# zengyf131/gswt_renderer

Measured on AMD Instinct MI355X. Metric: frames/sec @1920x1080, 32x32 Wang-tile grid, higher is better.
Workload: dtype f32

## Files before the change

gswt_renderer_amd/_lib.py:

```python
from __future__ import annotations

import ctypes as C
import os

_HERE = os.path.dirname(os.path.abspath(__file__))
LIB_PATH = os.environ.get("GSWT_HIP_LIB") or os.path.join(_HERE, "lib", "libgswt_hip.so")

GSWT_OK = 0
GSWT_ERR_BAD_ARG = -1
GSWT_ERR_CAPACITY = -2
GSWT_ERR_HIP = -3
GSWT_ERR_STATE = -4
GSWT_ERR_RCCL = -6
GSWT_COMM_ID_BYTES = 128
GSWT_ORDER_REFERENCE = 0
GSWT_ORDER_DEPTH = 1
GSWT_OPT_NO_LOD_PREFILTER = 1
GSWT_OPT_DEBUG_VARYINGS = 2
GSWT_OPT_SEGMENT = 3
GSWT_DEFAULT_SEGMENT = 1536
GSWT_OPT_DEBUG_FLAGS = 4
GSWT_OPT_TIMING = 5
GSWT_OPT_PAIR_CAP = 6
GSWT_OPT_NO_MERGE_REUSE = 7
GSWT_OPT_DEFER_SWAP = 8
GSWT_OPT_GRAPH = 9
GSWT_OPT_STRICT_VS = 10
GSWT_OPT_DEPTH_PASSES = 12
GSWT_OPT_COMPOSITE = 13
GSWT_OPT_DEPTH_SORT = 14
GSWT_OPT_NO_CHUNK_CULL = 15
GSWT_OPT_ITEM_ORDER = 16
GSWT_OPT_PROJECTION = 17
GSWT_PROJECTION_PERSPECTIVE, GSWT_PROJECTION_ORTHO = 0, 1
GSWT_OPT_ANTIALIAS = 18
GSWT_SCENE_TEX = 0
GSWT_SCENE_RAW_DEPTH = 1
GSWT_SCENE_RAW_TABLES = 2
GSWT_SCENE_STATIC_LIST = 3
GSWT_SCENE_STATIC_BOXES = 4
GSWT_SCENE_LISTS = 5
GSWT_SCENE_BOUNDS = 6
GSWT_SHARD_ROWS = 0
GSWT_SHARD_COLUMNS = 1
GSWT_OUT_RGBA32F = 0
GSWT_OUT_RGBA8_UNORM = 1
GSWT_OUT_BGRA8_UNORM = 2
GSWT_VIDEO_NV12 = 16
GSWT_VIDEO_I420 = 17
GSWT_PROXY_SRC_RGBA8 = 0
GSWT_PROXY_SRC_RGBA16 = 1


class CameraUniforms(C.Structure):
    _fields_ = [("projection", C.c_float * 16), ("view", C.c_float * 16), ("focal", C.c_float * 2),
                ("viewport", C.c_float * 2), ("htan_fov", C.c_float * 4), ("cam_pos", C.c_float * 4)]


class SceneUniforms(C.Structure):
    _fields_ = [("splat_scale", C.c_float), ("tile_width", C.c_float), ("use_clip", C.c_uint32),
                ("clip_height", C.c_float), ("surface_type", C.c_uint32), ("sphere_radius", C.c_float),
                ("point_cloud_radius", C.c_float), ("transition_width_ratio", C.c_float),
                ("num_lod", C.c_uint32), ("draw_mode", C.c_uint32), ("map_half_wh", C.c_uint32 * 2),
                ("center_coord", C.c_int32 * 2), ("_pad0", C.c_uint32 * 2),
                ("transition_dist_vec", C.c_float * 16), ("height_map_scale", C.c_float * 4),
                ("scene_scale", C.c_float * 4)]


# ... 187 lines not shown
```

gswt_renderer_amd/csrc/gswt_api.hip:

```cpp
#include "gswt_ctx.h"
#include "host/gswt_surface.h"

#include <algorithm>
#include <limits>
#include <memory>

using namespace gswt;


static int finish_frame(gswt_ctx* c, FrameSlot& sl);

void gswt::collect_slot(gswt_ctx* c, FrameSlot& sl)
{
    if (!sl.pending || sl.collected) return;
    sl.collected_rc = finish_frame(c, sl);
    sl.collected_timings = c->timings;
    sl.collected = true;
}

hipError_t gswt::collect_pending(gswt_ctx* c)
{
    for (auto& sl : c->slots) collect_slot(c, sl);
    return sync_all(c);
}
// ... 94 lines not shown
    if (c->own_stream && c->stream) hipStreamDestroy(c->stream);
    if (hip_stream) { c->stream = (hipStream_t)hip_stream; c->own_stream = false; return GSWT_OK; }
    c->stream = nullptr; c->own_stream = true;
    hipSetDevice(c->device);
    HIP_TRY(c, hipStreamCreateWithFlags(&c->stream, hipStreamNonBlocking));
    return GSWT_OK;
} GSWT_CATCH

int gswt_set_option(gswt_ctx* c, int key, int value)
try {
    if (!c) return GSWT_ERR_BAD_ARG;
    switch (key) {
    case GSWT_OPT_NO_LOD_PREFILTER: c->opt.no_prefilter = value; c->draws_ready = false; return GSWT_OK;
    case GSWT_OPT_DEBUG_VARYINGS: c->opt.debug_varyings = value; return GSWT_OK;
    case GSWT_OPT_DEBUG_FLAGS:
        if (value != 0) return fail(c, GSWT_ERR_BAD_ARG, "GSWT_OPT_DEBUG_FLAGS is reserved: only 0 is accepted");
        return GSWT_OK;
    case GSWT_OPT_TIMING: c->opt.timing = value; return GSWT_OK;
    case GSWT_OPT_NO_MERGE_REUSE: c->opt.no_merge_reuse = value; return GSWT_OK;
    case GSWT_OPT_DEFER_SWAP: c->opt.defer_swap = value; return GSWT_OK;
    case GSWT_OPT_GRAPH: c->opt.graph = value; return GSWT_OK;
    case GSWT_OPT_STRICT_VS: c->opt.strict_vs = value != 0; return GSWT_OK;
    case GSWT_OPT_PROJECTION:
        if (value != 0 && value != 1) return fail(c, GSWT_ERR_BAD_ARG, "GSWT_OPT_PROJECTION: 0 (perspective) or 1 (orthographic), not %d", value);
        c->opt.projection = value; return GSWT_OK;
    case GSWT_OPT_ANTIALIAS:
        if (value < 0 || value > 4096) return fail(c, GSWT_ERR_BAD_ARG, "GSWT_OPT_ANTIALIAS: 0 (off) or 1..4096 (filter variance in 1/1024 px^2), not %d", value);
        c->opt.antialias = value; return GSWT_OK;
    case GSWT_OPT_COMPOSITE:
        if (value < 0 || value > 2) return fail(c, GSWT_ERR_BAD_ARG, "unknown compositor variant %d", value);
        c->opt.composite = value; return GSWT_OK;
    case GSWT_OPT_NO_CHUNK_CULL: c->opt.no_chunk_cull = value != 0; return GSWT_OK;
    case GSWT_OPT_ITEM_ORDER: c->opt.item_order = value != 0; return GSWT_OK;
    case GSWT_OPT_DEPTH_SORT:
        if (value < 0 || value > 2) return fail(c, GSWT_ERR_BAD_ARG, "GSWT_OPT_DEPTH_SORT: 0 (auto), 1 (global passes) or 2 (tile-local)");
        c->opt.depth_sort = value; c->depth_max_tile_len = 0;
        return GSWT_OK;
    case GSWT_OPT_DEPTH_PASSES:
        if (value < 1 || value > 4) return fail(c, GSWT_ERR_BAD_ARG, "depth-sort passes must be 1..4");
        c->depth_passes = (uint32_t)value; c->depth_passes_low_run = 0;
        return GSWT_OK;
    case GSWT_OPT_PAIR_CAP:
        if (value < 0) return fail(c, GSWT_ERR_BAD_ARG, "pair capacity must be >= 0");
        c->opt.fixed_pair_cap = value > 0; if (value > 0) c->pair_cap = (uint32_t)value;
        return GSWT_OK;
    case GSWT_OPT_SEGMENT:
        if (value < 256 || value % 256) return fail(c, GSWT_ERR_BAD_ARG, "segment must be a positive multiple of 256");
        c->opt.segment = value; return GSWT_OK;
    default: return fail(c, GSWT_ERR_BAD_ARG, "unknown option %d", key);
    }
} GSWT_CATCH

int gswt_set_atmosphere(gswt_ctx* c, const gswt_atmosphere* a)
try {
    if (!c) return GSWT_ERR_BAD_ARG;
    if (!a) { c->atm = gswt_atmosphere{}; return GSWT_OK; }
    const float inf = std::numeric_limits<float>::infinity();
    const struct { const char* name; float v; } fields[] = {
        {"fade_start", a->fade_start}, {"fade_end", a->fade_end}, {"fog_density", a->fog_density}, {"fog_start", a->fog_start},
        {"fog_max", a->fog_max}, {"fog_color[0]", a->fog_color[0]}, {"fog_color[1]", a->fog_color[1]}, {"fog_color[2]", a->fog_color[2]}};
    for (const auto& fd : fields)
        if (!(std::fabs(fd.v) < inf)) return fail(c, GSWT_ERR_BAD_ARG, "gswt_set_atmosphere: %s = %g is not finite", fd.name, fd.v);
    if (a->fade_start != 0.0f || a->fade_end != 0.0f) {
        if (!(a->fade_start >= 0.0f)) return fail(c, GSWT_ERR_BAD_ARG, "gswt_set_atmosphere: fade_start = %g, not >= 0", a->fade_start);
        if (!(a->fade_end > a->fade_start))
            return fail(c, GSWT_ERR_BAD_ARG, "gswt_set_atmosphere: fade_end = %g, not above fade_start = %g", a->fade_end, a->fade_start);
// ... 218 lines not shown
    if (!sl.live_cnt.p) { HIP_TRY(c, sl.live_cnt.ensure(16 * kSuperStride)); HIP_TRY(c, hipMemsetAsync(sl.live_cnt.p, 0, sl.live_cnt.cap * 4, sl.stream)); }
    HIP_TRY(c, sl.draw_culled.ensure_roomy((size_t)D.n_draws + 1));
    HIP_TRY(c, sl.cell_culled.ensure((size_t)b.n_cells + 1));
    if (a.su.draw_mode != 0u) HIP_TRY(c, sl.col_f.ensure(n_slots_all + 1));
    if (need_depths) HIP_TRY(c, sl.depths.ensure(n_slots_all + 1));
    if (c->opt.debug_varyings) HIP_TRY(c, c->dbg.ensure((size_t)D.n_entries + 1));
    const size_t range_words = 2 * (nt + 1), list_words = tile_depth_list_words(nt);
    auto uint2s = [](size_t words) { return (words + 1) / 2 + 1; };
    HIP_TRY(c, sl.ranges.ensure(range_words / 2 + 2 * uint2s(list_words)));
    b.n_zero_ranges = (uint32_t)(range_words + list_words + 1);
    const size_t counter_words = 16, n_super = (size_t)D.n_chunks / 256 + 1;
    const size_t super_words = (2 * (size_t)kSuperStride + 1) * n_super;
    const size_t rw_pair = radix_ws_words(cap, key_bits), rw_depth = depth_bits ? radix_ws_words(cap, depth_bits) : 0;
    HIP_TRY(c, sl.ghist.ensure_roomy(counter_words + super_words + rw_pair + rw_depth + 16));
    b.n_zero_head = (uint32_t)(counter_words + super_words + radix_ws_zero_words(cap, key_bits));
    b.n_zero_depth = depth_bits ? (uint32_t)radix_ws_zero_words(cap, depth_bits) : 0u;
    HIP_TRY(c, sl.keys_a.ensure_roomy((size_t)cap + 1)); HIP_TRY(c, sl.keys_b.ensure_roomy((size_t)cap + 1));
    HIP_TRY(c, sl.vals_a.ensure_roomy((size_t)cap + 1)); HIP_TRY(c, sl.vals_b.ensure_roomy((size_t)cap + 1));
    if (depth_order) { HIP_TRY(c, sl.aux_a.ensure_roomy((size_t)cap + 1)); HIP_TRY(c, sl.aux_b.ensure_roomy((size_t)cap + 1)); }
    HIP_TRY(c, sl.item_base.ensure_roomy(nt + 2));
    HIP_TRY(c, sl.partials.ensure_roomy((nt + cap / seg + 1) * 256));
    if (a.d_out_depth) HIP_TRY(c, sl.partials_z.ensure_roomy((nt + cap / seg + 1) * 256));
    if (a.d_out_pick) HIP_TRY(c, sl.partials_pick.ensure_roomy((nt + cap / seg + 1) * 256));
    HIP_TRY(c, sl.item_tab.ensure_roomy(nt + cap / seg + 2));

    b.draws = D.draws; b.n_chunks = D.n_chunks; b.chunk_tab = D.chunk_tab.p; b.chunk_tab_xcd = D.chunk_tab_xcd.p;
    b.static_list = c->static_list.p; b.merged_list = D.merged_list.p; b.merged_map = D.merged_map.p;
    b.tex = c->tex.p; b.hmap = c->hmap.p; b.boxes = c->static_boxes.p;
    b.bg_rgba = a.d_bg; b.bg_depth = a.d_bgd; b.out = a.d_out; b.out_depth = a.d_out_depth; b.host_counters = sl.hc_dev;
    b.out_pick = reinterpret_cast<uint4*>(a.d_out_pick);
    b.n_tiles = (uint32_t)n_tiles; b.pair_cap = cap; b.seg = seg;
    b.rects = sl.rects.p; b.recs = sl.recs.p; b.depths = need_depths ? sl.depths.p : nullptr; b.col_f = sl.col_f.p; b.dbg = c->dbg.p;
    b.draw_culled = sl.draw_culled.p; b.cell_culled = sl.cell_culled.p;
    b.live_cnt = sl.live_cnt.p; b.live_cid = sl.live_cid.p; b.live_tab = sl.live_tab.p; b.block_sums = sl.block_sums.p;
    b.counters = reinterpret_cast<unsigned long long*>(sl.ghist.p);
    b.krange = reinterpret_cast<uint32_t*>(b.counters + 5);
    b.super_sums = sl.ghist.p + counter_words;
    b.radix_pair = b.super_sums + super_words;
    b.radix_depth = b.radix_pair + rw_pair;
    b.keys_a = sl.keys_a.p; b.keys_b = sl.keys_b.p; b.vals_a = sl.vals_a.p; b.vals_b = sl.vals_b.p; b.aux_a = sl.aux_a.p; b.aux_b = sl.aux_b.p;
    b.ranges = sl.ranges.p;
    b.long_tiles = reinterpret_cast<uint32_t*>(sl.ranges.p) + range_words;
    b.item_base = sl.item_base.p; b.item_tab = sl.item_tab.p; b.partials = sl.partials.p; b.partials_z = a.d_out_depth ? sl.partials_z.p : nullptr;
    b.partials_pick = a.d_out_pick ? sl.partials_pick.p : nullptr;
    const bool time_pick = a.d_out_pick != nullptr && c->opt.timing >= 1;
    b.ev_pick_begin = time_pick ? sl.ev[kEvPickBegin] : nullptr; b.ev_pick_end = time_pick ? sl.ev[kEvPickEnd] : nullptr;
    sl.pick_timed = time_pick && n_tiles > 0;
    return GSWT_OK;
}

static int emit_and_sort(gswt_ctx* c, const FrameSlot& sl, const Frame& f, const FrameBufs& b, int key_bits, const uint32_t** sorted)
{
    hipStream_t s = sl.stream;
    const uint32_t n_launch = c->opt.debug_varyings ? 0u : sl.n_launch_eff;
    const unsigned long long* const n_pairs = b.counters + 1;
    const uint32_t cap = b.pair_cap;
    if (sl.args.cfg.order_mode != GSWT_ORDER_DEPTH) {
        launch_emit(s, f, b, b.keys_a, nullptr, nullptr, n_launch);
        if (c->opt.timing >= 2) HIP_TRY(c, hipEventRecord(sl.ev[kEvEmitted], s));
        const int where = launch_sort(s, b.keys_a, b.vals_a, b.keys_b, b.vals_b, cap, n_pairs, key_bits, b.radix_pair, b.ranges);
        *sorted = where ? b.vals_b : b.vals_a;
    } else if (sl.depth_local) {
        launch_emit(s, f, b, b.keys_a, b.aux_a, nullptr, n_launch);
        if (c->opt.timing >= 2) HIP_TRY(c, hipEventRecord(sl.ev[kEvEmitted], s));
        const int where = launch_sort(s, b.keys_a, b.vals_a, b.keys_b, b.vals_b, cap, n_pairs, key_bits, b.radix_pair, b.ranges, nullptr, b.aux_a, b.aux_b);
        uint32_t* const vals = where ? b.vals_b : b.vals_a;
        launch_tile_depth_sort(s, b.ranges, vals, where ? b.aux_b : b.aux_a, where ? b.vals_a : b.vals_b, where ? b.aux_a : b.aux_b, (int)b.n_tiles,
// ... 35 lines not shown
    sl.depth_passes = depth_order ? std::min<uint32_t>(std::max<uint32_t>(c->depth_passes, 1u), 4u) : 0u;
    sl.depth_local = depth_order && c->opt.depth_sort != 1;
    if (depth_order) (sl.depth_local ? c->stat_depth_local : c->stat_depth_global)++;
    FrameBufs b;
    int rc = plan_frame_buffers(c, sl, D, f, n_tiles, sl.cap, key_bits, sl.depth_local ? 0 : 8 * (int)sl.depth_passes, b);
    if (rc != GSWT_OK) return rc;
    if (hipStreamQuery(c->stream) != hipSuccess) {
        HIP_TRY(c, hipEventRecord(sl.ev_in, c->stream));
        HIP_TRY(c, hipStreamWaitEvent(s, sl.ev_in, 0));
    }
    if (D.ev_up && D.ev_up_pending && !D.built) {
        if (hipEventQuery(D.ev_up) == hipSuccess) D.built = true;
        else HIP_TRY(c, hipStreamWaitEvent(s, D.ev_up, 0));
    }
    if (g.world > 1 && out_px > 0) HIP_TRY(c, hipMemsetAsync(a.d_out, 0, g.bytes, s));
    if (g.world > 1 && out_px > 0 && a.d_out_depth) HIP_TRY(c, hipMemsetAsync(a.d_out_depth, 0, out_px * sizeof(float), s));
    if (g.world > 1 && out_px > 0 && a.d_out_pick) HIP_TRY(c, hipMemsetAsync(a.d_out_pick, 0, out_px * sizeof(gswt_pick), s));
    const bool use_graph = c->opt.graph != 0 && c->opt.timing == 0 && !dbg && n_tiles > 0 && sl.hc_dev != nullptr;
    struct RecorderScope {
        explicit RecorderScope(GraphRec* r) { if (r) { r->n = 0; r->overflow = false; } graph_recorder() = r; }
        ~RecorderScope() { graph_recorder() = nullptr; }
    } recorder_scope(use_graph ? &sl.grec : nullptr);
    hipEvent_t* ev = sl.ev;
    if (c->opt.timing >= 1) HIP_TRY(c, hipEventRecord(ev[kEvStart], s));
    launch_cull(s, f, b, c->opt.no_chunk_cull == 0 && !dbg);
    {
        uint64_t eff = D.n_launch;
        if (!dbg && !sl.full_grid && c->live_hint) {
            const uint64_t cut = 8ull * ((uint64_t)c->live_hint + c->live_hint / 2 + 256);
            if (cut * 2 <= eff) eff = cut;
        }
        sl.n_launch_eff = (uint32_t)eff;
    }
    launch_project(s, f, b, sl.n_launch_eff, dbg, a.strict_vs, a.ortho);
    if (c->opt.timing >= 2) HIP_TRY(c, hipEventRecord(ev[kEvProjected], s));
    const uint32_t* vals = nullptr;
    rc = emit_and_sort(c, sl, f, b, key_bits, &vals);
    if (rc != GSWT_OK) return rc;
    if (c->opt.timing >= 2) HIP_TRY(c, hipEventRecord(ev[kEvSorted], s));
    if (c->opt.timing >= 2) HIP_TRY(c, hipEventRecord(ev[kEvRanges], s));
    launch_composite(s, f, b, vals, out_rows, c->opt.composite, depth_order && !sl.depth_local ? b.krange : nullptr, sl.depth_passes, depth_order,
                     c->opt.item_order != 0, c->opt.timing >= 1 ? ev[kEvCompositeBegin] : nullptr, c->opt.timing >= 1 ? ev[kEvCompositeEnd] : nullptr,
                     (int)a.cfg.out_format);
    c->last_n_tiles = (uint32_t)n_tiles;
    c->last_slot = (int)(&sl - c->slots);
    if (c->opt.timing >= 1) HIP_TRY(c, hipEventRecord(ev[kEvEnd], s));
    if (use_graph) {
        graph_recorder() = nullptr;
        const int grc = replay_graph(c, sl);
        if (grc != GSWT_OK) return grc;
    }
    HIP_TRY(c, hipGetLastError());
    if (n_tiles == 0 || !sl.hc_dev) HIP_TRY(c, hipMemcpyAsync(sl.hc, b.counters, 5 * sizeof(unsigned long long), hipMemcpyDeviceToHost, s));
    HIP_TRY(c, hipEventRecord(ev[kEvDone], s));
    sl.timing_level = c->opt.timing;
    return GSWT_OK;
}

static int finish_frame(gswt_ctx* c, FrameSlot& sl)
{
    for (int attempt = 0;; attempt++) {
        HIP_TRY(c, hipEventSynchronize(sl.ev[kEvDone]));
        const unsigned long long P64 = sl.hc[1];
        if (P64 >= 0xFFFFFF00ull) return fail(c, GSWT_ERR_CAPACITY, "gswt_render: %llu pairs exceed 2^32", P64);
        if (sl.hc[3] == 0 && P64 <= sl.cap) break;
        if (attempt >= 3) return fail(c, GSWT_ERR_CAPACITY, "gswt_render: pair capacity did not converge");
// ... 349 lines not shown
```

gswt_renderer_amd/csrc/gswt_ctx.h:

```cpp
#pragma once

#include "../../include/gswt_hip.h"
#include "gswt_device.h"

#include <cstdarg>
#include <cstdio>
#include <cstdlib>
#include <cstring>
#include <new>
#include <string>
#include <utility>
#include <vector>

namespace gswt {

template <typename T>
struct DevBuf {
    T* p = nullptr;
    size_t cap = 0;
    DevBuf() = default;
    DevBuf(DevBuf&& o) noexcept : p(std::exchange(o.p, nullptr)), cap(std::exchange(o.cap, 0)) {}
    DevBuf& operator=(DevBuf&& o) noexcept { std::swap(p, o.p); std::swap(cap, o.cap); return *this; }
    ~DevBuf() { release(); }
    hipError_t ensure(size_t n)
// ... 105 lines not shown
    float4* d_out = nullptr;
    float* d_out_depth = nullptr;
    gswt_pick* d_out_pick = nullptr;
    bool strict_vs = false;
    bool ortho = false;
    float aa_s = 0.0f;
    Atmo atm = {};
};

enum FrameEvent { kEvStart, kEvProjected, kEvEmitted, kEvSorted, kEvRanges, kEvEnd, kEvCompositeBegin, kEvCompositeEnd, kEvPickBegin, kEvPickEnd, kEvDone, kFrameEvents };

struct FrameSlot {
    hipStream_t stream = nullptr;
    hipEvent_t ev[kFrameEvents] = {};
    hipEvent_t ev_in = nullptr;
    hipEvent_t ev_gather = nullptr;
    bool gather_recorded = false;
    unsigned long long seq = 0;
    unsigned long long* hc = nullptr;
    unsigned long long* hc_dev = nullptr;
    bool pending = false;
    bool collected = false;
    int collected_rc = 0;
    gswt_timings collected_timings = {};
    FrameArgs args;
    int set = 0;
    uint32_t cap = 0;
    int n_tiles = 0;
    int timing_level = 0;
    DevBuf<uint2> rects;
    DevBuf<Rec> recs;
    DevBuf<uint4> live_tab;
    DevBuf<uint32_t> live_cnt;
    DevBuf<uint32_t> live_cid;
    DevBuf<uint32_t> cell_culled;
    DevBuf<uint32_t> block_sums, draw_culled, keys_a, keys_b, vals_a, vals_b, ghist;
    DevBuf<uint2> ranges;
    DevBuf<uint32_t> item_base;
    DevBuf<uint4> item_tab;
    DevBuf<uint32_t> aux_a, aux_b;
    uint32_t depth_passes = 0;
    bool depth_local = false;
    bool full_grid = false;
    uint32_t n_launch_eff = 0;
    DevBuf<float4> partials;
    DevBuf<float> partials_z;
    DevBuf<uint2> partials_pick;
    bool pick_timed = false;
    DevBuf<float4> col_f;
    DevBuf<float> depths;
    GraphRec grec;
    hipGraph_t graph = nullptr;
    hipGraphExec_t graph_exec = nullptr;
    hipGraphNode_t graph_nodes[kGraphMaxNodes] = {};
    GraphNodeRec graph_last[kGraphMaxNodes];
    uint32_t graph_n = 0;
    void release_graph()
    {
        if (graph_exec) hipGraphExecDestroy(graph_exec);
        if (graph) hipGraphDestroy(graph);
        graph_exec = nullptr; graph = nullptr; graph_n = 0;
    }
};

struct Options {
    int no_prefilter = 0;
    int debug_varyings = 0;
    int timing = 2;
    int segment = 1536;
    int fixed_pair_cap = 0;
    int defer_swap = 0;
    int graph = 0;
    int strict_vs = 1;
    int projection = 0;
    int antialias = 0;
    int composite = 0;
    int no_chunk_cull = 0;
    int no_merge_reuse = 0;
    int depth_sort = 0;
    int item_order = 0;
};

}

struct gswt_ctx {
    int device = 0;
    gswt::FrameSlot slots[gswt::kFrameSlots];
    unsigned long long frame_seq = 0;
    hipStream_t stream = nullptr;
    bool own_stream = true;
    std::string err;
    gswt::Options opt;
    gswt_atmosphere atm = {};
    gswt::DevBuf<uint4> tex;
    size_t n_splats = 0;
    float loc_lo[3] = {}, loc_hi[3] = {}, loc_max_trace = 0.0f;
    gswt::DevBuf<uint32_t> static_list;
    gswt::DevBuf<float> static_boxes;
    std::vector<gswt::ListRef> lists;
    size_t static_n = 0, boxes_n = 0;
    int n_lod = 0, n_tile = 0, n_view = 0;
    bool scene_ready = false;
    gswt::DevBuf<float> hmap;
    int hm_w = 0, hm_h = 0;
    float hm_min = 0.f, hm_max = 0.f, hm_du = 0.f, hm_dv = 0.f;
    gswt::DevBuf<float4> sky_faces;
    int sky_size = 0, sky_equi = 0;
    gswt::DevBuf<float4> proxy_tex;
    int proxy_size = 0, proxy_mips = 0, proxy_grid_dim = 2048;
    uint32_t proxy_mip_off[16] = {};
    gswt::DrawSet sets[gswt::kDrawSets];
    int cur_set = 0;
    int latest_set = 0;
// ... 117 lines not shown
```

gswt_renderer_amd/csrc/gswt_device.h:

```cpp
#pragma once
#include <hip/hip_runtime.h>
#include <hip/hip_ext.h>
#include <hip/hip_fp16.h>
#include <stdint.h>
#include <string.h>
#include <type_traits>

namespace gswt {

constexpr int kTile = 16;
constexpr int kChunk = 256;
__host__ __device__ inline void chunk_entry_range(uint32_t count, uint32_t k, uint32_t& lo, uint32_t& hi)
{
    hi = count - k * (uint32_t)kChunk;
    lo = hi > (uint32_t)kChunk ? hi - (uint32_t)kChunk : 0u;
}
constexpr uint32_t kLodShift = 28;
constexpr uint32_t kIdxMask = (1u << kLodShift) - 1u;
constexpr int kOutF32 = 0, kOutRGBA8 = 1, kOutBGRA8 = 2;
constexpr int kOutNV12 = 16, kOutI420 = 17;
constexpr bool out_is_video(int out_format) { return out_format == kOutNV12 || out_format == kOutI420; }
inline size_t out_image_bytes(int out_format, int rows, int out_w)
{
    if (rows < 0 || out_w < 0) return 0;
// ... 206 lines not shown
    do {                                                                                                 \
        if ((E0) && (E1) && !graph_recorder() && kernel_events_enabled())                                \
            hipExtLaunchKernelGGL(K, G, B, 0, S, E0, E1, 0, __VA_ARGS__);                                \
        else {                                                                                           \
            if (E0) hipEventRecord(E0, S);                                                               \
            GSWT_LAUNCH(K, G, B, S, __VA_ARGS__);                                                        \
            if (E1) hipEventRecord(E1, S);                                                               \
        }                                                                                                \
    } while (0)

struct FrameBufs {
    const DrawDev* draws;
    const uint2 *chunk_tab, *chunk_tab_xcd;
    const uint32_t *static_list, *merged_list, *merged_map;
    const uint4* tex;
    const float *hmap, *boxes;
    const float4* bg_rgba; const float* bg_depth; float4* out;
    float* out_depth;
    uint4* out_pick;
    unsigned long long* host_counters;
    uint32_t n_chunks, n_cells, n_tiles, pair_cap, seg;
    uint2* rects; Rec* recs; float4* col_f; Varyings* dbg;
    float* depths;
    uint32_t *draw_culled, *cell_culled, *live_cnt, *live_cid, *block_sums; uint4* live_tab;
    unsigned long long* counters;
    uint32_t *krange, *super_sums, *radix_pair, *radix_depth;
    uint32_t *keys_a, *keys_b, *vals_a, *vals_b, *aux_a, *aux_b;
    uint2* ranges; uint32_t* long_tiles;
    uint32_t* item_base; uint4* item_tab; float4* partials;
    float* partials_z;
    uint2* partials_pick;
    hipEvent_t ev_pick_begin, ev_pick_end;
    uint32_t n_zero_head, n_zero_ranges, n_zero_depth;
};

void launch_chunk_tabs(hipStream_t s, const DrawDev* draws, const uint32_t* xcd_first, uint32_t n_draws, uint2* chunk_tab, uint2* chunk_tab_xcd,
                       const uint64_t per_xcd[8], uint64_t longest);
void launch_merge_build(hipStream_t s, const MergeSeg* segs, uint32_t n_segs, const uint2* blocks, uint32_t n_blocks, MergeGroup* groups, uint32_t n_groups,
                        const int32_t* raw, uint32_t n_total, const unsigned long long* n_total_dev, uint32_t* ka, uint32_t* va,
                        uint32_t* kb, uint32_t* vb, uint32_t* radix_ws, int group_bits, uint32_t* merged_list, uint32_t* merged_map);
int launch_scene_sort(hipStream_t s, const MergeSeg* segs, const uint2* blocks, uint32_t n_blocks, MergeGroup* groups, const int32_t* raw,
                      uint32_t n_total, const unsigned long long* n_total_dev, uint32_t* ka, uint32_t* va, uint32_t* kb, uint32_t* vb,
                      uint32_t* radix_ws, int group_bits);
void launch_scene_tex(hipStream_t s, const uint4* rows, uint32_t n, uint4* tex, int32_t* bounds);
void launch_scene_raw(hipStream_t s, const uint4* rows, uint32_t n, const uint32_t* moff, const uint32_t* cnt, uint32_t n_lt, const SceneViews& vps,
                      int32_t* raw);
void launch_scene_scatter(hipStream_t s, const MergeSeg* segs, uint32_t n_segs, const MergeGroup* groups, const uint32_t* sorted_keys,
                          const uint32_t* sorted_vals, uint32_t n_total, uint32_t* arena, uint32_t arena_n);
void launch_scene_self(hipStream_t s, const SceneList* lists, uint32_t n_lists, uint32_t lists_per_lod, uint32_t* arena);
void launch_scene_boxes(hipStream_t s, const SceneList* lists, uint32_t n_lists, uint32_t n_boxes, const uint32_t* arena, const uint4* tex,
                        uint32_t n_splats, float* boxes);
void launch_merge_copy(hipStream_t s, const MergeCopy* jobs, const uint2* blocks, uint32_t n_blocks, const uint2* remap, const MergeSources& src,
                       uint32_t* new_list, uint32_t* new_map);

void launch_cull(hipStream_t s, const Frame& f, const FrameBufs& b, bool chunk_cull);
void launch_project(hipStream_t s, const Frame& f, const FrameBufs& b, uint32_t n_launch, bool debug, bool strict, bool ortho);
void launch_emit(hipStream_t s, const Frame& f, const FrameBufs& b, uint32_t* keys, uint32_t* dkeys, uint32_t* krange, uint32_t n_launch);
void launch_composite(hipStream_t s, const Frame& f, const FrameBufs& b, const uint32_t* vals, int out_rows, int variant, const uint32_t* krange,
                      uint32_t depth_passes, bool report_max, bool heavy_first, hipEvent_t ev_begin, hipEvent_t ev_end, int out_format);
void launch_totals(hipStream_t s, uint32_t* super_sums, uint32_t n_super, unsigned long long* counters, uint32_t pair_cap);

size_t radix_ws_words(uint32_t n_cap, int key_bits);
size_t radix_ws_zero_words(uint32_t n_cap, int key_bits);
int launch_sort(hipStream_t s, uint32_t* keys_a, uint32_t* vals_a, uint32_t* keys_b, uint32_t* vals_b, uint32_t n_cap,
                const unsigned long long* n_ptr, int key_bits, uint32_t* ws, uint2* ranges = nullptr, const uint32_t* krange = nullptr,
                uint32_t* aux_a = nullptr, uint32_t* aux_b = nullptr);
// ... 18 lines not shown
```

gswt_renderer_amd/csrc/gswt_kernels.hip:

```cpp
#include "gswt_device_fn.h"

namespace gswt {

template <int CTRL, int ROW_MASK>
__device__ __forceinline__ uint32_t dpp_or_zero(uint32_t x)
{
    return (uint32_t)__builtin_amdgcn_update_dpp(0, (int)x, CTRL, ROW_MASK, 0xF, true);
}
__device__ __forceinline__ uint32_t wave_incl_scan(uint32_t v, uint32_t lane)
{
    (void)lane;
    v += dpp_or_zero<0x111, 0xF>(v);
    v += dpp_or_zero<0x112, 0xF>(v);
    v += dpp_or_zero<0x114, 0xF>(v);
    v += dpp_or_zero<0x118, 0xF>(v);
    v += dpp_or_zero<0x142, 0xA>(v);
    v += dpp_or_zero<0x143, 0xC>(v);
    return v;
}
template <int CTRL, int ROW_MASK>
__device__ __forceinline__ uint32_t dpp_or_self(uint32_t x)
{
    return (uint32_t)__builtin_amdgcn_update_dpp((int)x, (int)x, CTRL, ROW_MASK, 0xF, false);
}
// ... 799 lines not shown
}

__device__ __forceinline__ uint32_t block_excl_scan(uint32_t v, uint32_t* s_w , uint32_t* total)
{
    const uint32_t lane = threadIdx.x & 63u, w = threadIdx.x >> 6;
    uint32_t inc = wave_incl_scan(v, lane);
    if (lane == 63u) s_w[w] = inc;
    __syncthreads();
    uint32_t base = 0;
    for (uint32_t i = 0; i < w; i++) base += s_w[i];
    *total = s_w[0] + s_w[1] + s_w[2] + s_w[3];
    __syncthreads();
    return base + inc - v;
}

constexpr uint32_t kEmitGroup = 4;

__device__ __forceinline__ uint32_t block_scan_and_sum(uint32_t v, uint32_t r, uint32_t* s_w , uint32_t* v_total, uint32_t* r_total)
{
    const uint32_t lane = threadIdx.x & 63u, w = threadIdx.x >> 6;
    const uint32_t inc = wave_incl_scan(v, lane);
    r = wave_sum(r);
    if (lane == 63u) s_w[w] = inc;
    if (lane == 0u) s_w[4u + w] = r;
    __syncthreads();
    uint32_t base = 0;
    for (uint32_t i = 0; i < w; i++) base += s_w[i];
    *v_total = s_w[0] + s_w[1] + s_w[2] + s_w[3];
    *r_total = s_w[4] + s_w[5] + s_w[6] + s_w[7];
    __syncthreads();
    return base + inc - v;
}

template <bool DEPTH, bool TAB>
__global__ __launch_bounds__(256) void k_emit(const Frame f, const uint2* __restrict__ rects,
                                              const uint32_t* __restrict__ block_sums, const uint32_t* __restrict__ super_excl,
                                              uint32_t n_chunks, uint32_t pair_cap, unsigned long long* __restrict__ counters,
                                              uint32_t* __restrict__ keys, uint32_t* __restrict__ vals,
                                              const float* __restrict__ depths, uint32_t* __restrict__ dkeys, uint32_t* __restrict__ krange,
                                              const uint32_t* __restrict__ live_cnt2, const uint32_t* __restrict__ live_cid)
{
    __shared__ uint32_t s_w[8];
    __shared__ uint32_t s_mn[DEPTH ? 4 : 1], s_mx[DEPTH ? 4 : 1];
#ifdef GSWT_TRACE
    const bool tr_on = threadIdx.x == 0 && blockIdx.x < 8192u;
    const uint32_t tr_item = 81920u + blockIdx.x;
    uint32_t tr_live = 0, tr_pairs = 0;
    GSWT_TR(0, GSWT_NOW())
    GSWT_TR(2, 0ull)
#endif
    uint32_t cid[kEmitGroup], sums[kEmitGroup], bs[kEmitGroup], sbase[kEmitGroup];
    uint2 rcs[kEmitGroup];
    float dep[kEmitGroup];
    uint32_t kmn = 0xFFFFFFFFu, kmx = 0u;
    uint32_t n_mine;
    if (TAB) {
        const uint32_t x = blockIdx.x & 7u, k0 = (blockIdx.x >> 3) * kEmitGroup;
        const uint32_t n_live = live_cnt2[x * kSuperStride];
        if (k0 >= n_live) return;
        n_mine = min(kEmitGroup, n_live - k0);
#pragma unroll
        for (uint32_t k = 0; k < kEmitGroup; k++) cid[k] = min(live_cid[(size_t)min(k0 + k, n_live - 1u) * 8u + x], n_chunks - 1u);
    } else {
        const uint32_t c0 = blockIdx.x * kEmitGroup;
        n_mine = min(kEmitGroup, n_chunks - c0);
#pragma unroll
        for (uint32_t k = 0; k < kEmitGroup; k++) cid[k] = min(c0 + k, n_chunks - 1u);
    }
#pragma unroll
    for (uint32_t k = 0; k < kEmitGroup; k++) {
        sums[k] = block_sums[cid[k]];
        bs[k] = block_sums[min((cid[k] & ~255u) + threadIdx.x, cid[k])];
        sbase[k] = super_excl[cid[k] >> 8];
        rcs[k] = rects[(size_t)cid[k] * 256u + threadIdx.x];
        dep[k] = DEPTH ? depths[(size_t)cid[k] * 256u + threadIdx.x] : 0.0f;
    }
    uint32_t any = 0;
#pragma unroll
    for (uint32_t k = 0; k < kEmitGroup; k++) { if (k >= n_mine) sums[k] = 0u; any |= sums[k]; }
#ifdef GSWT_TRACE
    { unsigned long long sink = sums[0] + bs[0] + sbase[3] + rcs[0].x + rcs[3].y; asm volatile("" :: "v"(sink)); }
    GSWT_TR(1, GSWT_NOW())
    for (uint32_t k = 0; k < kEmitGroup; k++) { tr_live += sums[k] ? 1u : 0u; tr_pairs += sums[k]; }
    GSWT_TR(3, tr_live)
    GSWT_TR(4, tr_pairs)
    if (any == 0u) { GSWT_TR(2, GSWT_NOW()) }
#endif
    if (any == 0u) return;
    const int sc = f.shard_count <= 1 ? 1 : f.shard_count;
#pragma unroll
    for (uint32_t k = 0; k < kEmitGroup; k++) {
        if (sums[k] == 0u) continue;
        const uint2 rc = rcs[k];
        const uint32_t slot = cid[k] * 256u + threadIdx.x;
        const int tx0 = rc.x & 0xFFFFu, tx1 = rc.x >> 16, ty0 = rc.y & 0xFFFFu, ty1 = rc.y >> 16;
        uint32_t count = 0;
        if (tx1 >= tx0) count = (uint32_t)((tx1 - tx0 + 1) * owned_rows(ty0, ty1, f.shard_index, f.shard_count));
        uint32_t tot, chunk_base;
        uint32_t off = block_scan_and_sum(count, (cid[k] & ~255u) + threadIdx.x < cid[k] ? bs[k] : 0u, s_w, &tot, &chunk_base);
        chunk_base += sbase[k];
        off += chunk_base;
        if ((unsigned long long)chunk_base + tot > (unsigned long long)pair_cap) {
            if (threadIdx.x == 0) atomicOr(&counters[3], 1ull);
            return;
        }
        if (count == 0) continue;
        const uint32_t dkey = __float_as_uint(dep[k] + 0.0f);
        if (DEPTH) { kmn = min(kmn, dkey); kmx = max(kmx, dkey); }
        if (sc > 1) {
            for (int ty = ty0 + ((f.shard_index - ty0 % sc) + sc) % sc; ty <= ty1; ty += sc) {
                const uint32_t row = (uint32_t)(ty / sc) * (uint32_t)f.tiles_x;
                for (int tx = tx0; tx <= tx1; tx++) {
                    keys[off] = row + (uint32_t)(tx - f.col0);
                    vals[off] = slot;
                    if (DEPTH) dkeys[off] = dkey;
                    off++;
                }
            }
        } else {
            for (int ty = ty0; ty <= ty1; ty++) {
                const uint32_t row = (uint32_t)ty * (uint32_t)f.tiles_x;
                for (int tx = tx0; tx <= tx1; tx++) {
                    keys[off] = row + (uint32_t)(tx - f.col0);
                    vals[off] = slot;
                    if (DEPTH) dkeys[off] = dkey;
                    off++;
                }
            }
        }
    }
    GSWT_TR(2, GSWT_NOW())
    if (DEPTH && krange) {
// ... 1367 lines not shown
}

void launch_cull(hipStream_t s, const Frame& f, const FrameBufs& b, bool chunk_cull)
{
    uint32_t grid = (b.n_chunks + 255u) / 256u;
    if (grid < 32) grid = 32;
    GSWT_LAUNCH(k_cull, dim3(grid), dim3(256), s, f, b.draws, b.draw_culled, b.cell_culled, b.n_cells, reinterpret_cast<uint32_t*>(b.counters), b.n_zero_head,
                reinterpret_cast<uint32_t*>(b.ranges), b.n_zero_ranges, b.block_sums, b.n_chunks, b.radix_depth, b.n_zero_depth,
                b.chunk_tab, b.n_chunks, b.boxes, chunk_cull && b.boxes ? 1u : 0u, b.live_cnt, b.live_tab, b.live_cid);
}

void launch_project(hipStream_t s, const Frame& f, const FrameBufs& b, uint32_t n_launch, bool debug, bool strict, bool ortho)
{
    if (b.n_chunks == 0) return;
    const uint32_t n_super = b.n_chunks / 256u + 1u;
    const bool full = f.surface_type == 2u || f.draw_mode != 0u;
#define GSWT_LAUNCH_PROJECT_S(D, F, S, O, A, M)                                                                                  \
    GSWT_LAUNCH((k_project<D, F, S, O, A, M>), dim3(n_launch), dim3(256), s, f, b.draws, b.chunk_tab_xcd, b.static_list, b.merged_list, \
                b.merged_map, b.tex, b.hmap, b.draw_culled, b.cell_culled, b.live_cnt, b.live_tab, b.rects, b.recs, b.depths, b.block_sums, \
                b.super_sums, n_super, b.dbg, b.col_f)
    const bool aa = f.aa_s > 0.0f, atm = f.atm.fade_end > 0.0f || f.atm.fog_density > 0.0f;
#define GSWT_LAUNCH_PROJECT_M(D, F, O, A) do { if (atm) GSWT_LAUNCH_PROJECT_S(D, F, true, O, A, true); else GSWT_LAUNCH_PROJECT_S(D, F, true, O, A, false); } while (0)
#define GSWT_LAUNCH_PROJECT_A(D, F, O) do { if (aa) GSWT_LAUNCH_PROJECT_M(D, F, O, true); else GSWT_LAUNCH_PROJECT_M(D, F, O, false); } while (0)
#define GSWT_LAUNCH_PROJECT(D, F) do { if (ortho) GSWT_LAUNCH_PROJECT_A(D, F, true); else if (strict) GSWT_LAUNCH_PROJECT_A(D, F, false); \
                                       else GSWT_LAUNCH_PROJECT_S(D, F, false, false, false, false); } while (0)
    if (debug && full) { GSWT_LAUNCH_PROJECT(true, true); }
    else if (debug) { GSWT_LAUNCH_PROJECT(true, false); }
    else if (full) { GSWT_LAUNCH_PROJECT(false, true); }
    else { GSWT_LAUNCH_PROJECT(false, false); }
#undef GSWT_LAUNCH_PROJECT
#undef GSWT_LAUNCH_PROJECT_A
#undef GSWT_LAUNCH_PROJECT_M
#undef GSWT_LAUNCH_PROJECT_S
    GSWT_LAUNCH(k_totals, dim3(1), dim3(256), s, b.super_sums, n_super, b.counters, b.super_sums + 2u * kSuperStride * n_super, b.pair_cap, b.live_cnt, n_launch / 8u);
}

void launch_emit(hipStream_t s, const Frame& f, const FrameBufs& b, uint32_t* keys, uint32_t* dkeys, uint32_t* krange, uint32_t n_launch)
{
    const uint32_t n_chunks = b.n_chunks, pair_cap = b.pair_cap;
    if (n_chunks == 0) return;
    const uint32_t n_super = n_chunks / 256u + 1u;
    const uint32_t* const excl = b.super_sums + 2u * kSuperStride * n_super;
    const float* const no_f = nullptr; uint32_t* const no_u = nullptr;
    const uint32_t* const cnt2 = n_launch ? b.live_cnt + 8u * kSuperStride : nullptr;
    const uint32_t* const cid = n_launch ? b.live_cid : nullptr;
    const dim3 grid(n_launch ? ((n_launch / 8u + kEmitGroup - 1u) / kEmitGroup) * 8u : (n_chunks + kEmitGroup - 1u) / kEmitGroup);
#define GSWT_LAUNCH_EMIT(D, L)                                                                                                 \
    GSWT_LAUNCH((k_emit<D, L>), grid, dim3(256), s, f, b.rects, b.block_sums, excl, n_chunks, pair_cap, b.counters, keys, b.vals_a, \
                D ? b.depths : no_f, D ? dkeys : no_u, D ? krange : no_u, cnt2, cid)
    if (n_launch) { if (dkeys) GSWT_LAUNCH_EMIT(true, true); else GSWT_LAUNCH_EMIT(false, true); }
    else if (dkeys) GSWT_LAUNCH_EMIT(true, false);
    else GSWT_LAUNCH_EMIT(false, false);
#undef GSWT_LAUNCH_EMIT
}

size_t radix_ws_words(uint32_t n_cap, int key_bits)
{
    const uint32_t nblk = (n_cap + kSortBlock - 1) / kSortBlock, nsup = (nblk >> kSupShift) + 1;
    const int passes = (key_bits + 7) / 8;
    return (size_t)passes * ((size_t)256 * nblk + (size_t)256 * nsup + 256);
}
size_t radix_ws_zero_words(uint32_t n_cap, int key_bits)
{
    const uint32_t nblk = (n_cap + kSortBlock - 1) / kSortBlock, nsup = (nblk >> kSupShift) + 1;
    const int passes = (key_bits + 7) / 8;
    return (size_t)passes * ((size_t)256 * nsup + 256);
}

int launch_sort(hipStream_t s, uint32_t* keys_a, uint32_t* vals_a, uint32_t* keys_b, uint32_t* vals_b, uint32_t n_cap,
                const unsigned long long* n_ptr, int key_bits, uint32_t* ws, uint2* ranges, const uint32_t* krange, uint32_t* aux_a, uint32_t* aux_b)
{
    if (n_cap == 0) return 0;
    const uint32_t nblk = (n_cap + kSortBlock - 1) / kSortBlock, nsup = (nblk >> kSupShift) + 1;
    const int threads = n_cap <= kSortWideMax ? 512 : 256;
    int cur = 0;
    const int passes = (key_bits + 7) / 8;
    uint32_t* hist_rows = ws + (size_t)passes * ((size_t)256 * nsup + 256);
    for (int shift = 0; shift < key_bits; shift += 8) {
        uint32_t nbits = (uint32_t)((key_bits - shift) < 8 ? (key_bits - shift) : 8);
        uint32_t mask = (1u << nbits) - 1u;
        uint32_t* gsup = ws; uint32_t* gtot = gsup + (size_t)256 * nsup;
        ws = gtot + 256;
        uint32_t* ghist = hist_rows;
        hist_rows += (size_t)256 * nblk;
        uint32_t* ki = cur ? keys_b : keys_a; uint32_t* vi = cur ? vals_b : vals_a;
// ... 178 lines not shown
```

include/gswt_hip.h:

```cpp
#ifndef GSWT_HIP_H
#define GSWT_HIP_H

#include <stddef.h>
#include <stdint.h>

#ifdef __cplusplus
extern "C" {
#endif

#define GSWT_API __attribute__((visibility("default")))

typedef struct gswt_ctx gswt_ctx;

enum {
    GSWT_OK = 0,
    GSWT_ERR_BAD_ARG = -1,
    GSWT_ERR_CAPACITY = -2,
    GSWT_ERR_HIP = -3,
    GSWT_ERR_STATE = -4,
    GSWT_ERR_RCCL = -6
};

enum { GSWT_ORDER_REFERENCE = 0, GSWT_ORDER_DEPTH = 1 };

// ... 86 lines not shown
typedef struct {
    float ms_project, ms_scan, ms_emit, ms_sort, ms_ranges, ms_composite, ms_total;
    uint32_t n_draws;
    uint64_t n_instanced;
    uint64_t n_visible;
    uint64_t n_pairs;
    uint32_t n_tiles;
    uint32_t _pad;
    float ms_composite_kernel;
    float ms_pick_resolve;
} gswt_timings;


GSWT_API int gswt_create(int device_id, gswt_ctx **out);
GSWT_API void gswt_destroy(gswt_ctx *ctx);
GSWT_API const char *gswt_last_error(const gswt_ctx *ctx);
GSWT_API int gswt_set_stream(gswt_ctx *ctx, void *hip_stream);

enum { GSWT_OPT_NO_LOD_PREFILTER = 1, GSWT_OPT_DEBUG_VARYINGS = 2,
       GSWT_OPT_SEGMENT = 3 ,
       GSWT_OPT_DEBUG_FLAGS = 4 ,
       GSWT_OPT_TIMING = 5 ,
       GSWT_OPT_PAIR_CAP = 6 ,
       GSWT_OPT_NO_MERGE_REUSE = 7 ,
       GSWT_OPT_DEFER_SWAP = 8 ,
       GSWT_OPT_GRAPH = 9 ,
       GSWT_OPT_STRICT_VS = 10 ,
       GSWT_OPT_DEPTH_PASSES = 12 ,
       GSWT_OPT_COMPOSITE = 13 ,
       GSWT_OPT_DEPTH_SORT = 14 ,
       GSWT_OPT_NO_CHUNK_CULL = 15 ,
       GSWT_OPT_ITEM_ORDER = 16 ,
       GSWT_OPT_PROJECTION = 17 ,
       GSWT_OPT_ANTIALIAS = 18  };
GSWT_API int gswt_set_option(gswt_ctx *ctx, int key, int value);

typedef struct {
    float fade_start, fade_end;
    float fog_density;
    float fog_start;
    float fog_max;
    float fog_color[3];
} gswt_atmosphere;
GSWT_API int gswt_set_atmosphere(gswt_ctx *ctx, const gswt_atmosphere *a);

GSWT_API int gswt_upload_scene(gswt_ctx *ctx, const uint32_t *tex_data, size_t n_splats,
                               const gswt_base_list *lists, int n_lod, int n_tile, int n_view);

GSWT_API int gswt_configure(gswt_ctx *ctx, const float *height_map, int hm_w, int hm_h);

GSWT_API int gswt_set_draws(gswt_ctx *ctx, const gswt_draw *draws, int n_draws,
                            const uint32_t *merged_gs_index, const uint32_t *merged_map_id,
                            const uint32_t *merged_lod_id, size_t n_merged);

typedef struct {
    uint32_t view_id;
    uint32_t first_member;
    uint32_t n_members;
    uint32_t _pad;
} gswt_merge_group;
typedef struct {
    uint32_t map_index;
    uint32_t lod, tile;
    int32_t other_lod;
} gswt_merge_member;
GSWT_API int gswt_upload_raw_depth(gswt_ctx *ctx, const int32_t *const *raw_depth ,
                                   const uint32_t *counts ,
// ... 218 lines not shown
```

rust/src/gswt_hip_sys.rs:

```rust
#![allow(non_camel_case_types, dead_code)]
use std::os::raw::{c_char, c_int, c_uint, c_void};

pub const GSWT_OK: c_int = 0;
pub const GSWT_ERR_BAD_ARG: c_int = -1;
pub const GSWT_ERR_CAPACITY: c_int = -2;
pub const GSWT_ERR_HIP: c_int = -3;
pub const GSWT_ERR_STATE: c_int = -4;
pub const GSWT_ERR_RCCL: c_int = -6;
pub const GSWT_ORDER_REFERENCE: c_int = 0;
pub const GSWT_ORDER_DEPTH: c_int = 1;
pub const GSWT_SHARD_ROWS: c_int = 0;
pub const GSWT_SHARD_COLUMNS: c_int = 1;
pub const GSWT_OUT_RGBA32F: c_int = 0;
pub const GSWT_OUT_RGBA8_UNORM: c_int = 1;
pub const GSWT_OUT_BGRA8_UNORM: c_int = 2;
pub const GSWT_VIDEO_NV12: c_int = 16;
pub const GSWT_VIDEO_I420: c_int = 17;
pub const GSWT_OPT_NO_LOD_PREFILTER: c_int = 1;
pub const GSWT_OPT_DEBUG_VARYINGS: c_int = 2;
pub const GSWT_OPT_SEGMENT: c_int = 3;
pub const GSWT_OPT_DEBUG_FLAGS: c_int = 4;
pub const GSWT_OPT_TIMING: c_int = 5;
pub const GSWT_OPT_PAIR_CAP: c_int = 6;
pub const GSWT_OPT_NO_MERGE_REUSE: c_int = 7;
pub const GSWT_OPT_DEFER_SWAP: c_int = 8;
pub const GSWT_OPT_GRAPH: c_int = 9;
pub const GSWT_OPT_STRICT_VS: c_int = 10;
pub const GSWT_OPT_DEPTH_PASSES: c_int = 12;
pub const GSWT_OPT_COMPOSITE: c_int = 13;
pub const GSWT_OPT_DEPTH_SORT: c_int = 14;
pub const GSWT_OPT_NO_CHUNK_CULL: c_int = 15;
pub const GSWT_OPT_ITEM_ORDER: c_int = 16;
pub const GSWT_OPT_PROJECTION: c_int = 17;
pub const GSWT_OPT_ANTIALIAS: c_int = 18;
pub const GSWT_SCENE_TEX: c_int = 0;
pub const GSWT_SCENE_RAW_DEPTH: c_int = 1;
pub const GSWT_SCENE_RAW_TABLES: c_int = 2;
pub const GSWT_SCENE_STATIC_LIST: c_int = 3;
pub const GSWT_SCENE_STATIC_BOXES: c_int = 4;
pub const GSWT_SCENE_LISTS: c_int = 5;
pub const GSWT_SCENE_BOUNDS: c_int = 6;
pub const GSWT_PROXY_SRC_RGBA8: c_int = 0;
pub const GSWT_PROXY_SRC_RGBA16: c_int = 1;
pub const GSWT_COMM_ID_BYTES: c_int = 128;

#[repr(C)] pub struct GswtCtx { _private: [u8; 0] }
#[repr(C)] pub struct GswtWorker { _private: [u8; 0] }

#[repr(C)] #[derive(Clone, Copy)]
pub struct GswtCameraUniforms {
    pub projection: [f32; 16],
    pub view: [f32; 16],
    pub focal: [f32; 2],
    pub viewport: [f32; 2],
    pub htan_fov: [f32; 4],
    pub cam_pos: [f32; 4],
}

#[repr(C)] #[derive(Clone, Copy)]
pub struct GswtSceneUniforms {
    pub splat_scale: f32,
    pub tile_width: f32,
    pub use_clip: u32,
    pub clip_height: f32,
    pub surface_type: u32,
    pub sphere_radius: f32,
    pub point_cloud_radius: f32,
// ... 505 lines not shown
```

Baseline: 5572.

## Fold k_totals reduction into k_emit to drop a single-block launch

Removes the separate one-block k_totals launch by having k_emit compute the per-superblock prefix in each block and block 0 write the global pair/visible counters and overflow flag. Live counters are double-buffered so block 0 of emit can clear the other set instead of needing a memset. This cuts one serialized kernel launch per frame, at the cost of every emit block loading and scanning the super sums redundantly; it only applies when n_super <= 256 and can be disabled via a new option.

```diff
diff --git a/gswt_renderer_amd/_lib.py b/gswt_renderer_amd/_lib.py
--- a/gswt_renderer_amd/_lib.py
+++ b/gswt_renderer_amd/_lib.py
@@ -34,6 +34,7 @@
 GSWT_OPT_PROJECTION = 17
 GSWT_PROJECTION_PERSPECTIVE, GSWT_PROJECTION_ORTHO = 0, 1
 GSWT_OPT_ANTIALIAS = 18
+GSWT_OPT_CHAIN = 19
 GSWT_SCENE_TEX = 0
 GSWT_SCENE_RAW_DEPTH = 1
 GSWT_SCENE_RAW_TABLES = 2
diff --git a/gswt_renderer_amd/csrc/gswt_api.hip b/gswt_renderer_amd/csrc/gswt_api.hip
--- a/gswt_renderer_amd/csrc/gswt_api.hip
+++ b/gswt_renderer_amd/csrc/gswt_api.hip
@@ -150,6 +150,9 @@
         c->opt.composite = value; return GSWT_OK;
     case GSWT_OPT_NO_CHUNK_CULL: c->opt.no_chunk_cull = value != 0; return GSWT_OK;
     case GSWT_OPT_ITEM_ORDER: c->opt.item_order = value != 0; return GSWT_OK;
+    case GSWT_OPT_CHAIN:
+        if (value != 0 && value != 1) return fail(c, GSWT_ERR_BAD_ARG, "GSWT_OPT_CHAIN: 0 (k_totals folded into k_emit) or 1 (launched), not %d", value);
+        c->opt.chain = value; return GSWT_OK;
     case GSWT_OPT_DEPTH_SORT:
         if (value < 0 || value > 2) return fail(c, GSWT_ERR_BAD_ARG, "GSWT_OPT_DEPTH_SORT: 0 (auto), 1 (global passes) or 2 (tile-local)");
         c->opt.depth_sort = value; c->depth_max_tile_len = 0;
@@ -434,7 +437,17 @@
     b.n_tiles = (uint32_t)n_tiles; b.pair_cap = cap; b.seg = seg;
     b.rects = sl.rects.p; b.recs = sl.recs.p; b.depths = need_depths ? sl.depths.p : nullptr; b.col_f = sl.col_f.p; b.dbg = c->dbg.p;
     b.draw_culled = sl.draw_culled.p; b.cell_culled = sl.cell_culled.p;
-    b.live_cnt = sl.live_cnt.p; b.live_cid = sl.live_cid.p; b.live_tab = sl.live_tab.p; b.block_sums = sl.block_sums.p;
+    b.live_cid = sl.live_cid.p; b.live_tab = sl.live_tab.p; b.block_sums = sl.block_sums.p;
+    b.fold_totals = c->opt.chain == 0 && D.n_chunks != 0 && n_super <= 256;
+    if (b.fold_totals) {
+        b.live_cnt = sl.live_cnt.p + sl.live_set * 8u * kSuperStride;
+        b.live_clear = sl.live_cnt.p + (sl.live_set ^ 1u) * 8u * kSuperStride;
+        sl.live_set ^= 1u;
+    } else {
+        if (sl.live_set != 0u) { HIP_TRY(c, hipMemsetAsync(sl.live_cnt.p, 0, 16 * kSuperStride * 4, sl.stream)); sl.live_set = 0u; }
+        b.live_cnt = sl.live_cnt.p; b.live_clear = nullptr;
+    }
+    b.n_launch_project = 0u;
     b.counters = reinterpret_cast<unsigned long long*>(sl.ghist.p);
     b.krange = reinterpret_cast<uint32_t*>(b.counters + 5);
     b.super_sums = sl.ghist.p + counter_words;
@@ -536,6 +549,7 @@
         }
         sl.n_launch_eff = (uint32_t)eff;
     }
+    b.n_launch_project = sl.n_launch_eff;
     launch_project(s, f, b, sl.n_launch_eff, dbg, a.strict_vs, a.ortho);
     if (c->opt.timing >= 2) HIP_TRY(c, hipEventRecord(ev[kEvProjected], s));
     const uint32_t* vals = nullptr;
diff --git a/gswt_renderer_amd/csrc/gswt_ctx.h b/gswt_renderer_amd/csrc/gswt_ctx.h
--- a/gswt_renderer_amd/csrc/gswt_ctx.h
+++ b/gswt_renderer_amd/csrc/gswt_ctx.h
@@ -161,6 +161,7 @@
     DevBuf<Rec> recs;
     DevBuf<uint4> live_tab;
     DevBuf<uint32_t> live_cnt;
+    uint32_t live_set = 0;
     DevBuf<uint32_t> live_cid;
     DevBuf<uint32_t> cell_culled;
     DevBuf<uint32_t> block_sums, draw_culled, keys_a, keys_b, vals_a, vals_b, ghist;
@@ -208,6 +209,7 @@
     int no_merge_reuse = 0;
     int depth_sort = 0;
     int item_order = 0;
+    int chain = 0;
 };
 
 }
diff --git a/gswt_renderer_amd/csrc/gswt_device.h b/gswt_renderer_amd/csrc/gswt_device.h
--- a/gswt_renderer_amd/csrc/gswt_device.h
+++ b/gswt_renderer_amd/csrc/gswt_device.h
@@ -262,6 +262,8 @@
     uint2* partials_pick;
     hipEvent_t ev_pick_begin, ev_pick_end;
     uint32_t n_zero_head, n_zero_ranges, n_zero_depth;
+    bool fold_totals;
+    uint32_t* live_clear; uint32_t n_launch_project;
 };
 
 void launch_chunk_tabs(hipStream_t s, const DrawDev* draws, const uint32_t* xcd_first, uint32_t n_draws, uint2* chunk_tab, uint2* chunk_tab_xcd,
diff --git a/gswt_renderer_amd/csrc/gswt_kernels.hip b/gswt_renderer_amd/csrc/gswt_kernels.hip
--- a/gswt_renderer_amd/csrc/gswt_kernels.hip
+++ b/gswt_renderer_amd/csrc/gswt_kernels.hip
@@ -855,15 +855,45 @@
     return base + inc - v;
 }
 
-template <bool DEPTH, bool TAB>
+struct EmitFold { uint32_t* live_clear; uint32_t launched_per_xcd; };
+template <bool DEPTH, bool TAB, typename... FOLD>
 __global__ __launch_bounds__(256) void k_emit(const Frame f, const uint2* __restrict__ rects,
                                               const uint32_t* __restrict__ block_sums, const uint32_t* __restrict__ super_excl,
                                               uint32_t n_chunks, uint32_t pair_cap, unsigned long long* __restrict__ counters,
                                               uint32_t* __restrict__ keys, uint32_t* __restrict__ vals,
                                               const float* __restrict__ depths, uint32_t* __restrict__ dkeys, uint32_t* __restrict__ krange,
-                                              const uint32_t* __restrict__ live_cnt2, const uint32_t* __restrict__ live_cid)
-{
+                                              const uint32_t* __restrict__ live_cnt2, const uint32_t* __restrict__ live_cid, const FOLD... fold)
+{
+    constexpr bool kFold = sizeof...(FOLD) != 0;
     __shared__ uint32_t s_w[8];
+    uint32_t sp = 0;
+    if constexpr (kFold) {
+        const EmitFold fa = (fold, ...);
+        const uint32_t n_super = n_chunks / 256u + 1u;
+        const uint32_t* const super_sums = super_excl;
+        sp = super_sums[min(threadIdx.x, n_super - 1u) * kSuperStride];
+        if (threadIdx.x >= n_super) sp = 0u;
+        if (blockIdx.x == 0u) {
+            __shared__ unsigned long long s_p64[4];
+            __shared__ uint32_t s_vis[4];
+            uint32_t vv = super_sums[(n_super + min(threadIdx.x, n_super - 1u)) * kSuperStride];
+            if (threadIdx.x >= n_super) vv = 0u;
+            uint32_t lv = 0;
+            if (threadIdx.x < 8u) { lv = live_cnt2[threadIdx.x * kSuperStride]; fa.live_clear[threadIdx.x * kSuperStride] = 0u; }
+            if (threadIdx.x < 64u) for (int o = 4; o > 0; o >>= 1) lv = max(lv, (uint32_t)__shfl_xor((int)lv, o, 64));
+            unsigned long long p64 = sp;
+            for (int off = 32; off > 0; off >>= 1) p64 += __shfl_down(p64, off, 64);
+            vv = wave_sum(vv);
+            if ((threadIdx.x & 63u) == 0u) { s_p64[threadIdx.x >> 6] = p64; s_vis[threadIdx.x >> 6] = vv; }
+            __syncthreads();
+            if (threadIdx.x == 0u) {
+                const unsigned long long pairs = s_p64[0] + s_p64[1] + s_p64[2] + s_p64[3];
+                counters[1] = pairs; counters[0] = (unsigned long long)s_vis[0] + s_vis[1] + s_vis[2] + s_vis[3];
+                counters[4] = lv;
+                if (pairs > (unsigned long long)pair_cap || lv > fa.launched_per_xcd) atomicOr(&counters[3], 1ull);
+            }
+        }
+    }
     __shared__ uint32_t s_mn[DEPTH ? 4 : 1], s_mx[DEPTH ? 4 : 1];
 #ifdef GSWT_TRACE
     const bool tr_on = threadIdx.x == 0 && blockIdx.x < 8192u;
@@ -894,6 +924,8 @@
     for (uint32_t k = 0; k < kEmitGroup; k++) {
         sums[k] = block_sums[cid[k]];
         bs[k] = block_sums[min((cid[k] & ~255u) + threadIdx.x, cid[k])];
+        if constexpr (kFold) sbase[k] = 0u;
+        else
         sbase[k] = super_excl[cid[k] >> 8];
         rcs[k] = rects[(size_t)cid[k] * 256u + threadIdx.x];
         dep[k] = DEPTH ? depths[(size_t)cid[k] * 256u + threadIdx.x] : 0.0f;
@@ -920,7 +952,7 @@
         uint32_t count = 0;
         if (tx1 >= tx0) count = (uint32_t)((tx1 - tx0 + 1) * owned_rows(ty0, ty1, f.shard_index, f.shard_count));
         uint32_t tot, chunk_base;
-        uint32_t off = block_scan_and_sum(count, (cid[k] & ~255u) + threadIdx.x < cid[k] ? bs[k] : 0u, s_w, &tot, &chunk_base);
+        uint32_t off = block_scan_and_sum(count, ((cid[k] & ~255u) + threadIdx.x < cid[k] ? bs[k] : 0u) + (kFold && threadIdx.x < (cid[k] >> 8) ? sp : 0u), s_w, &tot, &chunk_base);
         chunk_base += sbase[k];
         off += chunk_base;
         if ((unsigned long long)chunk_base + tot > (unsigned long long)pair_cap) {
@@ -2354,7 +2386,8 @@
 #undef GSWT_LAUNCH_PROJECT_A
 #undef GSWT_LAUNCH_PROJECT_M
 #undef GSWT_LAUNCH_PROJECT_S
-    GSWT_LAUNCH(k_totals, dim3(1), dim3(256), s, b.super_sums, n_super, b.counters, b.super_sums + 2u * kSuperStride * n_super, b.pair_cap, b.live_cnt, n_launch / 8u);
+    if (!b.fold_totals)
+        GSWT_LAUNCH(k_totals, dim3(1), dim3(256), s, b.super_sums, n_super, b.counters, b.super_sums + 2u * kSuperStride * n_super, b.pair_cap, b.live_cnt, n_launch / 8u);
 }
 
 void launch_emit(hipStream_t s, const Frame& f, const FrameBufs& b, uint32_t* keys, uint32_t* dkeys, uint32_t* krange, uint32_t n_launch)
@@ -2370,9 +2403,19 @@
 #define GSWT_LAUNCH_EMIT(D, L)                                                                                                 \
     GSWT_LAUNCH((k_emit<D, L>), grid, dim3(256), s, f, b.rects, b.block_sums, excl, n_chunks, pair_cap, b.counters, keys, b.vals_a, \
                 D ? b.depths : no_f, D ? dkeys : no_u, D ? krange : no_u, cnt2, cid)
-    if (n_launch) { if (dkeys) GSWT_LAUNCH_EMIT(true, true); else GSWT_LAUNCH_EMIT(false, true); }
+    const EmitFold fold = {b.live_clear, b.n_launch_project / 8u};
+#define GSWT_LAUNCH_EMIT_FOLD(D, L)                                                                                            \
+    GSWT_LAUNCH((k_emit<D, L, EmitFold>), grid, dim3(256), s, f, b.rects, b.block_sums, (const uint32_t*)b.super_sums, n_chunks, pair_cap, b.counters, keys, \
+                b.vals_a, D ? b.depths : no_f, D ? dkeys : no_u, D ? krange : no_u, (const uint32_t*)b.live_cnt, cid, fold)
+    if (b.fold_totals) {
+        if (n_launch) { if (dkeys) GSWT_LAUNCH_EMIT_FOLD(true, true); else GSWT_LAUNCH_EMIT_FOLD(false, true); }
+        else if (dkeys) GSWT_LAUNCH_EMIT_FOLD(true, false);
+        else GSWT_LAUNCH_EMIT_FOLD(false, false);
+    }
+    else if (n_launch) { if (dkeys) GSWT_LAUNCH_EMIT(true, true); else GSWT_LAUNCH_EMIT(false, true); }
     else if (dkeys) GSWT_LAUNCH_EMIT(true, false);
     else GSWT_LAUNCH_EMIT(false, false);
+#undef GSWT_LAUNCH_EMIT_FOLD
 #undef GSWT_LAUNCH_EMIT
 }
 
diff --git a/include/gswt_hip.h b/include/gswt_hip.h
--- a/include/gswt_hip.h
+++ b/include/gswt_hip.h
@@ -142,7 +142,8 @@
        GSWT_OPT_NO_CHUNK_CULL = 15 ,
        GSWT_OPT_ITEM_ORDER = 16 ,
        GSWT_OPT_PROJECTION = 17 ,
-       GSWT_OPT_ANTIALIAS = 18  };
+       GSWT_OPT_ANTIALIAS = 18 ,
+       GSWT_OPT_CHAIN = 19  };
 GSWT_API int gswt_set_option(gswt_ctx *ctx, int key, int value);
 
 typedef struct {
diff --git a/rust/src/gswt_hip_sys.rs b/rust/src/gswt_hip_sys.rs
--- a/rust/src/gswt_hip_sys.rs
+++ b/rust/src/gswt_hip_sys.rs
@@ -33,6 +33,7 @@
 pub const GSWT_OPT_ITEM_ORDER: c_int = 16;
 pub const GSWT_OPT_PROJECTION: c_int = 17;
 pub const GSWT_OPT_ANTIALIAS: c_int = 18;
+pub const GSWT_OPT_CHAIN: c_int = 19;
 pub const GSWT_SCENE_TEX: c_int = 0;
 pub const GSWT_SCENE_RAW_DEPTH: c_int = 1;
 pub const GSWT_SCENE_RAW_TABLES: c_int = 2;
```

Result: no change. 5604 (median of 6 runs) (+0.6%).
